# decadenza/SimpleStereo

Measured on AMD Instinct MI355X. Metric: disparity MPixels/s (H*W*nDisp per second), higher is better.
Workload: dtype f32

## Files before the change

simplestereo_amd/csrc/asw_exact_kernels.hip.h:

```cpp
#pragma once
#include "asw_shared.hip.h"
#include "lab_kernels.hip.h"
#include "glibc_math.hip.h"

namespace ssamd {

struct AswExactArgs {
    const PixRec *recL, *recR;
    const double *labL, *labR;
    const double *prox;
    u64 *keyL, *keyR;
    int16_t *disp;
    AswExactQueue q;
    AswExactQueue raw;
    double *ecost;
    u64 *costL, *costR;
    uint32_t *idxL, *idxR;
    uint32_t *wslotL, *wslotR;
    uint32_t *wpix;
    double *wtab;
    unsigned int wcap;
    int H, W, win, pad, minD, maxD, row0, rows;
    double gammaC;
};

__device__ __forceinline__ double exact_sqrt(double x)
{
#pragma clang fp contract(off)
    const double y0 = sqrt(x);
    if (!(y0 > 0.0) || !(y0 < 1.0e300)) return y0;
    const double e = fma(-y0, y0, x);
    return y0 + e / (2.0 * y0);
}

__global__ __launch_bounds__(256) void bgr2lab_f64_pair_kernel(const PixRec *__restrict__ recL, const PixRec *__restrict__ recR,
                                                               double *__restrict__ labL, double *__restrict__ labR, long long npix)
{
    SSAMD_LAB_TABLES_IN_LDS(T)
    long long q = (long long)blockIdx.x * blockDim.x + threadIdx.x;
    const long long stride = (long long)gridDim.x * blockDim.x;
    for (; q < 2 * npix; q += stride) {
        const bool right = q >= npix;
        const long long p = right ? q - npix : q;
        const uint32_t v = (right ? recR : recL)[p].bgrx;
        double L, a, b;
        bgr_to_lab_f64(v & 0xff, (v >> 8) & 0xff, (v >> 16) & 0xff, L, a, b, T);
        double *const o = (right ? labR : labL) + 3 * p;
        o[0] = L; o[1] = a; o[2] = b;
    }
}

__device__ __forceinline__ bool exact_overflowed(const AswExactArgs &A)
{
    return A.q.counter[0] > A.q.cap || (A.raw.entries && A.raw.counter[0] > A.raw.cap);
}

__global__ __launch_bounds__(256) void asw_exact_filter_kernel(const AswExactArgs A)
{
    const unsigned n = min(A.raw.counter[0], A.raw.cap);
    const unsigned nloop = (n + 255u) & ~255u;
    for (unsigned e0 = blockIdx.x * blockDim.x; e0 < nloop; e0 += gridDim.x * blockDim.x) {
        const unsigned e = e0 + threadIdx.x;
        unsigned s2 = 0;
        uint32_t pix = 0, rkey = 0xffffffffu;
        int d = 0;
        if (e < n) {
            const u64 ent = A.raw.entries[e];
            const uint32_t key = A.raw.ekeys[e];
            rkey = key;
            pix = (uint32_t)ent;
            d = (int)((ent >> 32) & 0xffff);
            const unsigned sides = (unsigned)(ent >> 48) & 3u;
            const uint32_t esc = 0xC0000000u - __float_as_uint(2.0f * A.q.sat_abs);
            if (sides & EXACT_SIDE_L) {
                const u64 g = A.keyL[pix];
                if ((int)(uint32_t)g != d && (uint32_t)(g >> 32) < esc && exact_near(key, (uint32_t)(g >> 32), A.q.tol, A.q.sat_abs, exact_zkey(A.win))) s2 |= EXACT_SIDE_L;
            }
            if ((sides & EXACT_SIDE_R) && A.keyR) {
                const u64 g = A.keyR[pix - (uint32_t)d];
                if ((uint32_t)g != pix % (uint32_t)A.W && (uint32_t)(g >> 32) < esc && exact_near(key, (uint32_t)(g >> 32), A.q.tol, A.q.sat_abs, exact_zkey(A.win))) s2 |= EXACT_SIDE_R;
            }
        }
        asw_exact_push_wave(A.q, s2 != 0, pix, d, s2, rkey);
    }
}

__global__ __launch_bounds__(256) void asw_exact_escalate_kernel(const AswExactArgs A)
{
    const AswExactQueue &Q = A.q;
    const uint32_t esc = 0xC0000000u - __float_as_uint(2.0f * Q.sat_abs);
    const long long n = (long long)A.rows * A.W;
    for (long long q = (long long)blockIdx.x * blockDim.x + threadIdx.x; q < n; q += (long long)gridDim.x * blockDim.x) {
        const int x = (int)(q % A.W);
        const u64 gl = A.keyL[q];
        if (gl != KEY_NONE && (uint32_t)(gl >> 32) >= esc) {
            const int dwin = (int)(uint32_t)gl, dhi = min(A.maxD, x);
            const int cnt = dhi - A.minD;
            if (cnt > 0) {
                unsigned slot = atomicAdd(Q.counter, (unsigned)cnt);
                for (int d = A.minD; d <= dhi; ++d)
                    if (d != dwin) {
                        if (slot < Q.cap) Q.entries[slot] = exact_entry((uint32_t)q, d, EXACT_SIDE_L);
                        ++slot;
                    }
                Q.flagL[q] = 1;
            }
        }
        if (A.keyR) {
            const u64 gr = A.keyR[q];
            if (gr != KEY_NONE && (uint32_t)(gr >> 32) >= esc) {
                const int xwin = (int)(uint32_t)gr;
                const int dhi = min(A.maxD, A.W - 1 - x), cnt = dhi - A.minD;
                if (cnt > 0) {
                    unsigned slot = atomicAdd(Q.counter, (unsigned)cnt);
                    for (int d = A.minD; d <= dhi; ++d)
                        if (x + d != xwin) {
                            if (slot < Q.cap) Q.entries[slot] = exact_entry((uint32_t)(q + d), d, EXACT_SIDE_R);
                            ++slot;
                        }
                    Q.flagR[q] = 1;
                }
            }
        }
    }
}

static constexpr int EXACT_ZSEG = 64, EXACT_ZWIN_MAX = 64;
__global__ __launch_bounds__(256) void asw_exact_zero_kernel(const AswExactArgs A)
{
    extern __shared__ __attribute__((aligned(16))) char zsmem[];
    const AswExactQueue &Q = A.q;
    const int W = A.W, H = A.H, win = A.win, p = A.pad;
    const int segs_per_row = (W + EXACT_ZSEG - 1) / EXACT_ZSEG;
    const int tid = threadIdx.x;
    const int TW = EXACT_ZSEG + 2 * p;
    uint32_t *const tA = reinterpret_cast<uint32_t *>(zsmem);
    uint32_t *const tB = tA + win * TW;
    __shared__ int s_idx[EXACT_ZSEG], s_state[EXACT_ZSEG];
    __shared__ int s_cur;
    for (long long seg = blockIdx.x; seg < (long long)A.rows * segs_per_row; seg += gridDim.x) {
        const int yr = (int)(seg / segs_per_row), x0 = (int)(seg - (long long)yr * segs_per_row) * EXACT_ZSEG, y = A.row0 + yr;
        if (!Q.zrow[yr]) continue;
        for (int side = 0; side < (A.keyR ? 2 : 1); ++side) {
            __syncthreads();
            if (tid < EXACT_ZSEG) {
                const int x = x0 + tid;
                bool z = false;
                int idx = 0;
                if (x < W) {
                    const long long q = (long long)yr * W + x;
                    if (side == 0) {
                        z = Q.zeroL[q] != 0;
                        if (z) {
                            if (A.keyL) { const u64 g = A.keyL[q]; z = g != KEY_NONE && (uint32_t)(g >> 32) == 0u; idx = (int)(uint32_t)g; }
                            else idx = (int)A.disp[q];
                        }
                    } else {
                        z = Q.zeroR[q] != 0;
                        if (z) { const u64 g = A.keyR[q]; z = g != KEY_NONE && (uint32_t)(g >> 32) == 0u; idx = (int)(uint32_t)g; }
                    }
                }
                s_idx[tid] = idx;
                s_state[tid] = z ? 1 : 0;
            }
            if (__syncthreads_or(tid < EXACT_ZSEG && s_state[tid] == 1) == 0) continue;
            if (win >= EXACT_ZWIN_MAX) {
                if (tid < EXACT_ZSEG && s_state[tid] == 1) s_state[tid] = 3;
            } else {
                const PixRec *const imgA = side ? A.recR : A.recL, *const imgB = side ? A.recL : A.recR;
                auto stage = [&](uint32_t *tile, const PixRec *img, int shift) {
                    for (int k0 = 0; k0 < win * TW; k0 += 8 * 256) {
                        uint32_t v[8];
#pragma unroll
                        for (int u = 0; u < 8; ++u) {
                            const int k = k0 + u * 256 + tid, i = k / TW, c = k - i * TW, ii = y - p + i, cc = x0 - p + c + shift;
                            v[u] = (k < win * TW && (unsigned)ii < (unsigned)H && (unsigned)cc < (unsigned)W) ? img[(size_t)ii * W + cc].bgrx : 0x80000000u;
                        }
#pragma unroll
                        for (int u = 0; u < 8; ++u) {
                            const int k = k0 + u * 256 + tid;
                            if (k < win * TW) tile[k] = v[u];
                        }
                    }
                };
                stage(tA, imgA, 0);
                for (;;) {
                    __syncthreads();
                    if (tid == 0) {
                        int cur = -1;
                        for (int k = 0; k < EXACT_ZSEG; ++k)
                            if (s_state[k] == 1) { cur = side ? s_idx[k] - (x0 + k) : s_idx[k]; break; }
                        s_cur = cur;
                    }
                    __syncthreads();
                    const int d = s_cur;
                    if (d < 0) break;
                    const int shift = side ? d : -d;
                    stage(tB, imgB, shift);
                    __syncthreads();
                    const int px = tid & (EXACT_ZSEG - 1), part = tid >> 6;
                    const bool mine = s_state[px] == 1 && (side ? s_idx[px] - (x0 + px) : s_idx[px]) == d;
                    bool nz = false;
                    if (mine) {
                        uint32_t acc = 0;
                        for (int i = part; i < win; i += 4) {
                            const uint32_t *const ra = tA + i * TW + px, *const rb = tB + i * TW + px;
#pragma unroll 8
                            for (int j = 0; j < win; ++j) {
                                const uint32_t a = ra[j], b = rb[j];
                                acc |= ((a | b) >> 31) ? 0u : (a ^ b);
                            }
                        }
                        nz = acc != 0u;
                    }
                    __syncthreads();
                    if (mine && part == 0) s_state[px] = 2;
                    __syncthreads();
                    if (mine && nz) s_state[px] = 3;
                }
            }
            __syncthreads();
            if (tid < EXACT_ZSEG && s_state[tid] == 3) {
                const int xq = x0 + tid, widx = s_idx[tid];
                const long long pq = (long long)yr * W + xq;
                if (side == 0) {
                    const int dhi = min(A.maxD, xq), cnt = dhi - A.minD;
                    if (cnt > 0) {
                        unsigned slot = atomicAdd(Q.counter, (unsigned)cnt);
                        for (int d = A.minD; d <= dhi; ++d)
                            if (d != widx) { if (slot < Q.cap) Q.entries[slot] = exact_entry((uint32_t)pq, d, EXACT_SIDE_L); ++slot; }
                        Q.flagL[pq] = 1;
                    }
                } else {
                    const int dhi = min(A.maxD, W - 1 - xq), cnt = dhi - A.minD;
                    if (cnt > 0) {
                        unsigned slot = atomicAdd(Q.counter, (unsigned)cnt);
                        for (int d = A.minD; d <= dhi; ++d)
                            if (xq + d != widx) { if (slot < Q.cap) Q.entries[slot] = exact_entry((uint32_t)(pq + d), d, EXACT_SIDE_R); ++slot; }
                        Q.flagR[pq] = 1;
                    }
                }
            }
        }
    }
}

__device__ __forceinline__ void exact_assign_wslot(const AswExactArgs &A, bool flagged, u64 mask, uint32_t pix, uint32_t side)
{
    if (mask == 0 || A.wcap == 0) return;
    const int leader = (int)__builtin_ctzll(mask);
    const unsigned lane = __builtin_amdgcn_mbcnt_hi(~0u, __builtin_amdgcn_mbcnt_lo(~0u, 0u));
    unsigned base = 0;
    if ((int)lane == leader) base = atomicAdd(A.q.counter + 6, (unsigned)__builtin_popcountll(mask));
    base = (unsigned)__builtin_amdgcn_readlane((int)base, leader);
    if (flagged) {
        const unsigned slot = base + (unsigned)__builtin_popcountll(mask & (((u64)1 << lane) - 1));
        (side ? A.wslotR : A.wslotL)[pix] = slot;
        if (slot < A.wcap) A.wpix[slot] = pix | (side << 31);
    }
}

__global__ __launch_bounds__(256) void asw_exact_winners_kernel(const AswExactArgs A)
{
    const AswExactQueue &Q = A.q;
    const long long n = (long long)A.rows * A.W;
    for (long long q0 = (long long)blockIdx.x * blockDim.x; q0 < n; q0 += (long long)gridDim.x * blockDim.x) {
        const long long q = q0 + threadIdx.x;
        const bool inb = q < n;
        const bool fl = inb && Q.flagL[q];
        if (fl) {
            A.costL[q] = ~0ull;
            A.idxL[q] = 0xffffffffu;
        }
        const int dwin = fl ? (A.keyL ? (int)(uint32_t)A.keyL[q] : (int)A.disp[q]) : 0;
        const u64 ml = __builtin_amdgcn_ballot_w64(fl);
        if (ml && fl && (int)__builtin_ctzll(ml) == (int)(threadIdx.x & 63)) atomicAdd(Q.counter + 1, (unsigned)__builtin_popcountll(ml));
        exact_assign_wslot(A, fl, ml, (uint32_t)q, 0u);
        asw_exact_push_wave(Q, fl, (uint32_t)q, dwin, EXACT_SIDE_L, fl && A.keyL ? (uint32_t)(A.keyL[q] >> 32) : 0xffffffffu);
        if (A.keyR) {
            const bool fr = inb && Q.flagR[q];
            int xl = 0, xr = 0;
            if (fr) {
                A.costR[q] = ~0ull;
                A.idxR[q] = 0xffffffffu;
                xr = (int)(q % A.W);
                xl = (int)(uint32_t)A.keyR[q];
            }
            const u64 mr = __builtin_amdgcn_ballot_w64(fr);
            if (mr && fr && (int)__builtin_ctzll(mr) == (int)(threadIdx.x & 63)) atomicAdd(Q.counter + 2, (unsigned)__builtin_popcountll(mr));
            exact_assign_wslot(A, fr, mr, (uint32_t)q, 1u);
            asw_exact_push_wave(Q, fr, (uint32_t)(q + (xl - xr)), xl - xr, EXACT_SIDE_R, fr ? (uint32_t)(A.keyR[q] >> 32) : 0xffffffffu);
        }
    }
}

__global__ __launch_bounds__(256) void asw_exact_wtab_kernel(const AswExactArgs A)
{
#pragma clang fp contract(off)
    __shared__ uint64_t s_exp[256];
    for (int k = threadIdx.x; k < 256; k += blockDim.x) s_exp[k] = gm_exp_tab[k];
    __syncthreads();
    if (exact_overflowed(A)) return;
    const unsigned n = min(A.q.counter[6], A.wcap);
    const int lane = threadIdx.x & 63, W = A.W, H = A.H, win = A.win, p = A.pad, win2 = win * win;
    for (unsigned slot = blockIdx.x * 4 + (threadIdx.x >> 6); slot < n; slot += gridDim.x * 4) {
        const uint32_t pw = A.wpix[slot], pix = pw & 0x7fffffffu;
        const double *const lab = (pw >> 31) ? A.labR : A.labL;
        const int yr = (int)(pix / (uint32_t)W), x = (int)(pix - (uint32_t)yr * (uint32_t)W), y = A.row0 + yr;
        const double *const c = lab + 3 * ((size_t)y * W + x);
        const double c0 = c[0], c1 = c[1], c2 = c[2];
        double *const out = A.wtab + (size_t)slot * win2;
        for (int t = lane; t < win2; t += 64) {
            const int i = t / win, j = t - i * win, ii = y - p + i, cc = x - p + j;
            double w = 0.0;
            if ((unsigned)ii < (unsigned)H && (unsigned)cc < (unsigned)W) {
                const double *const tp = lab + 3 * ((size_t)ii * W + cc);
                const double a0 = tp[0] - c0, a1 = tp[1] - c1, a2 = tp[2] - c2;
                w = A.prox[t] * glibc_exp_t(-exact_sqrt(a0 * a0 + a1 * a1 + a2 * a2) / A.gammaC, s_exp);
            }
            out[t] = w;
        }
    }
}

static constexpr int EXACT_WAVES = 4;
static constexpr int EXACT_CHUNK = 256;
__global__ __launch_bounds__(64 * EXACT_WAVES) void asw_exact_eval_kernel(const AswExactArgs A)
{
#pragma clang fp contract(off)
    __shared__ double s_w[EXACT_WAVES][EXACT_CHUNK], s_c[EXACT_WAVES][EXACT_CHUNK];
    __shared__ uint64_t s_exp[256];
    for (int k = threadIdx.x; k < 256; k += blockDim.x) s_exp[k] = gm_exp_tab[k];
    __syncthreads();
    if (exact_overflowed(A)) return;
    const int lane = threadIdx.x & 63, wv = threadIdx.x >> 6;
    double *const sw = s_w[wv], *const sc = s_c[wv];
    const unsigned n = min(A.q.counter[0], A.q.cap);
    const int W = A.W, H = A.H, win = A.win, p = A.pad;
    for (unsigned e = blockIdx.x * EXACT_WAVES + wv; e < n; e += gridDim.x * EXACT_WAVES) {
        const u64 ent = A.q.entries[e];
        const uint32_t pix = (uint32_t)ent;
        const int d = (int)((ent >> 32) & 0xffff);
        const unsigned sides = (unsigned)(ent >> 48) & 3u;
        const int yr = (int)(pix / (uint32_t)W), x = (int)(pix - (uint32_t)yr * (uint32_t)W);
        const int y = A.row0 + yr, xr = x - d;
        const double *const cl = A.labL + 3 * ((size_t)y * W + x), *const cr = A.labR + 3 * ((size_t)y * W + xr);
        const double cl0 = cl[0], cl1 = cl[1], cl2 = cl[2], cr0 = cr[0], cr1 = cr[1], cr2 = cr[2];
        const int jlo = max(0, p - xr), jhi = min(win, W + p - x), ncol = jhi - jlo;
        const int ilo = max(0, p - y), ihi = min(win, H + p - y);
        const int ntap = (ihi - ilo) * ncol;
        const uint32_t s1 = A.wcap && A.q.flagL && A.q.flagL[pix] ? A.wslotL[pix] : 0xffffffffu;
        const uint32_t s2 = A.wcap && A.q.flagR && A.q.flagR[pix - (uint32_t)d] ? A.wslotR[pix - (uint32_t)d] : 0xffffffffu;
        const double *const t1 = s1 < A.wcap ? A.wtab + (size_t)s1 * win * win : nullptr;
        const double *const t2 = s2 < A.wcap ? A.wtab + (size_t)s2 * win * win : nullptr;
        double acc = 0.0;
        bool all_zero = false;
        if ((unsigned)(ent >> 48) & EXACT_HINT_ZERO) {
            bool nz = false;
            for (int t = lane; t < ntap; t += 64) {
                const int q = t / ncol, i = ilo + q, j = jlo + (t - q * ncol);
                const int ii = y - p + i, jj = xr - p + j, kk = x - p + j;
                nz = nz || __builtin_amdgcn_sad_u8(A.recL[(size_t)ii * W + kk].bgrx, A.recR[(size_t)ii * W + jj].bgrx, 0u) != 0u;
            }
            all_zero = __builtin_amdgcn_ballot_w64(nz) == 0;
        }
        for (int t0 = 0; t0 < (all_zero ? 0 : ntap); t0 += EXACT_CHUNK) {
            const int nt = min(EXACT_CHUNK, ntap - t0);
            for (int t = lane; t < nt; t += 64) {
                const int q = (t0 + t) / ncol, i = ilo + q, j = jlo + (t0 + t - q * ncol);
                const int ii = y - p + i, jj = xr - p + j, kk = x - p + j;
                const double pr = A.prox[i * win + j];
                double w1, w2;
                if (t1) w1 = t1[i * win + j];
                else {
                    const double *const tl = A.labL + 3 * ((size_t)ii * W + kk);
                    const double a0 = tl[0] - cl0, a1 = tl[1] - cl1, a2 = tl[2] - cl2;
                    w1 = pr * glibc_exp_t(-exact_sqrt(a0 * a0 + a1 * a1 + a2 * a2) / A.gammaC, s_exp);
                }
                if (t2) w2 = t2[i * win + j];
                else {
                    const double *const tr = A.labR + 3 * ((size_t)ii * W + jj);
                    const double b0 = tr[0] - cr0, b1 = tr[1] - cr1, b2 = tr[2] - cr2;
                    w2 = pr * glibc_exp_t(-exact_sqrt(b0 * b0 + b1 * b1 + b2 * b2) / A.gammaC, s_exp);
                }
                const int tad = min(40, (int)__builtin_amdgcn_sad_u8(A.recL[(size_t)ii * W + kk].bgrx, A.recR[(size_t)ii * W + jj].bgrx, 0u));
                const double ww = w1 * w2;
                sw[t] = ww;
                sc[t] = ww * tad;
            }
            __builtin_amdgcn_wave_barrier();
            asm volatile("s_waitcnt lgkmcnt(0)" ::: "memory");
            if (lane < 2) {
                const double *const src = lane ? sw : sc;
                int t = 0;
                for (; t + 16 <= nt; t += 16) {
                    double v[16];
#pragma unroll
                    for (int u = 0; u < 16; ++u) v[u] = src[t + u];
#pragma unroll
                    for (int u = 0; u < 16; ++u) acc += v[u];
                }
                for (; t < nt; ++t) acc += src[t];
            }
            asm volatile("s_waitcnt lgkmcnt(0)" ::: "memory");
            __builtin_amdgcn_wave_barrier();
        }
        const double tot = __shfl(acc, 1);
        if (lane == 0) {
            const double c = all_zero ? 0.0 : acc / tot;
            A.ecost[e] = c;
            const u64 bits = (u64)__double_as_longlong(c);
            if (sides & EXACT_SIDE_L) atomicMin(A.costL + pix, bits);
            if (sides & EXACT_SIDE_R) atomicMin(A.costR + (pix - (uint32_t)d), bits);
        }
    }
}

__global__ __launch_bounds__(256) void asw_exact_resolve_kernel(const AswExactArgs A)
{
    if (exact_overflowed(A)) return;
    const unsigned n = A.q.counter[0];
    for (unsigned e = blockIdx.x * blockDim.x + threadIdx.x; e < n; e += gridDim.x * blockDim.x) {
        const u64 ent = A.q.entries[e];
        const uint32_t pix = (uint32_t)ent;
        const int d = (int)((ent >> 32) & 0xffff);
        const unsigned sides = (unsigned)(ent >> 48) & 3u;
        const u64 bits = (u64)__double_as_longlong(A.ecost[e]);
        if ((sides & EXACT_SIDE_L) && A.costL[pix] == bits) atomicMin(A.idxL + pix, (uint32_t)d);
        if ((sides & EXACT_SIDE_R) && A.costR[pix - (uint32_t)d] == bits) atomicMin(A.idxR + (pix - (uint32_t)d), pix % (uint32_t)A.W);
    }
}

__global__ __launch_bounds__(256) void asw_exact_patch_kernel(const AswExactArgs A)
{
    if (exact_overflowed(A)) return;
    const long long n = (long long)A.rows * A.W;
    for (long long q = (long long)blockIdx.x * blockDim.x + threadIdx.x; q < n; q += (long long)gridDim.x * blockDim.x) {
        if (A.q.flagL[q] && A.idxL[q] != 0xffffffffu) {
            if (A.keyL) A.keyL[q] = (A.keyL[q] & 0xffffffff00000000ull) | (u64)A.idxL[q];
            else A.disp[q] = (int16_t)A.idxL[q];
        }
        if (A.keyR && A.q.flagR[q] && A.idxR[q] != 0xffffffffu) A.keyR[q] = (A.keyR[q] & 0xffffffff00000000ull) | (u64)A.idxR[q];
    }
}

}
```

simplestereo_amd/csrc/host_asw_exact.h:

```cpp
namespace {
int get_prox64(Ctx &c, int win, double gammaP, hipStream_t s, const double **out);

int asw_exact_prepare(Ctx &c, int W, int rows, int win, int nD, double gammaC, bool consistent, bool direct, hipStream_t s,
                      AswExactQueue &q, AswExactQueue &raw, AswExactQueue &kernel_q)
{
    const size_t nout = (size_t)rows * W;
    if (nout >= ((size_t)1 << 32)) return fail(SSAMD_ELIMIT, "exact mode: more than 2^32 output pixels per call");
    const size_t all_cands = 2 * (nout * (size_t)nD + nout);
    size_t cap = std::min<size_t>(std::max<size_t>(4 * nout, std::min<size_t>(all_cands, (size_t)1 << 23)), (size_t)1 << 26);
    if (tune().exact_cap) cap = (size_t)tune().exact_cap;
    size_t rawcap = direct ? 0 : std::min<size_t>(std::max<size_t>(2 * nout, std::min<size_t>(all_cands, (size_t)1 << 23)), (size_t)1 << 26);
    if (!direct && tune().exact_cap) rawcap = std::max<size_t>(rawcap, cap);
    if (!direct && tune().exact_rawcap) rawcap = (size_t)tune().exact_rawcap;
    int rc;
    if ((rc = c.xqueue.reserve(cap * 8)) || (rc = c.xcost.reserve(cap * 8)) || (rc = c.xflags.reserve(64 + 4 * nout + (size_t)rows)) ||
        (rc = c.xslots.reserve(nout * 32)) || (rawcap && (rc = c.xraw.reserve(rawcap * 12))))
        return rc;
    c.xcap = (unsigned int)cap;
    c.xrawcap = (unsigned int)rawcap;
    HIP_TRY(hipMemsetAsync(c.xflags.ptr, 0, 64 + 4 * nout + (size_t)rows, s));
    q.entries = (u64 *)c.xqueue.ptr;
    q.ekeys = nullptr;
    q.counter = (unsigned int *)c.xflags.ptr;
    q.flagL = (unsigned char *)c.xflags.ptr + 64;
    q.flagR = consistent ? q.flagL + nout : nullptr;
    q.zeroL = q.flagL + 2 * nout;
    q.zeroR = consistent ? q.flagL + 3 * nout : nullptr;
    q.zrow = q.flagL + 4 * nout;
    q.W = (unsigned int)W;
    q.cap = (unsigned int)cap;
    q.tol = (uint32_t)std::min(1.0e6, (double)tune().exact_tol * std::max(1.0, 5.0 / gammaC) * std::max(1.0, win / 35.0));
    q.sat_abs = (float)(1.5 * 2.0 * 2.0 * ((double)win * win + 3.0) * 1.1102230246251565e-16 * 40.0);
    q.deep = 0xffffffffu;
    raw = AswExactQueue{};
    if (!direct) {
        raw = q;
        union { float f; uint32_t u; } sa; sa.f = q.sat_abs;
        raw.deep = 0xC0000000u - sa.u;
        raw.entries = (u64 *)c.xraw.ptr;
        raw.ekeys = (uint32_t *)((u64 *)c.xraw.ptr + rawcap);
        raw.counter = q.counter + 4;
        raw.flagL = raw.flagR = nullptr;
        raw.cap = (unsigned int)rawcap;
    }
    kernel_q = direct ? q : raw;
    return SSAMD_OK;
}

int asw_exact_pass(Ctx &c, const AswExactQueue &q, const AswExactQueue &raw, int H, int W, int row0, int rows, int win, int maxD, int minD, double gammaC, double gammaP,
                   bool consistent, bool direct, int16_t *d_disp, hipStream_t s)
{
    const int p = win / 2;
    const size_t nout = (size_t)rows * W, npix = (size_t)H * W;
    int rc;
    const double *d_prox = nullptr;
    if ((rc = get_prox64(c, win, gammaP, s, &d_prox))) return rc;
    if ((rc = c.xlabL.reserve(npix * 24)) || (rc = c.xlabR.reserve(npix * 24))) return rc;
    AswExactArgs x;
    x.recL = (const PixRec *)c.recL.ptr; x.recR = (const PixRec *)c.recR.ptr;
    x.labL = (const double *)c.xlabL.ptr; x.labR = (const double *)c.xlabR.ptr;
    x.prox = d_prox;
    x.keyL = direct ? nullptr : (u64 *)c.keyL.ptr; x.keyR = consistent ? (u64 *)c.keyR.ptr : nullptr;
    x.disp = d_disp;
    x.q = q;
    x.raw = raw;
    x.ecost = (double *)c.xcost.ptr;
    x.costL = (u64 *)c.xslots.ptr; x.costR = x.costL + nout;
    x.idxL = (uint32_t *)(x.costR + nout); x.idxR = x.idxL + nout;
    x.wslotL = x.idxR + nout; x.wslotR = x.wslotL + nout;
    {
        const size_t per = (size_t)win * win * 8;
        size_t wcap = std::min<size_t>(65536, ((size_t)64 << 20) / per);
        if (nout >= ((size_t)1 << 31)) wcap = 0;
        if (wcap && (rc = c.xwtab.reserve(wcap * 8 + wcap * per))) return rc;
        x.wcap = (unsigned int)wcap;
        x.wpix = (uint32_t *)c.xwtab.ptr;
        x.wtab = (double *)((char *)c.xwtab.ptr + wcap * 8);
    }
    x.H = H; x.W = W; x.win = win; x.pad = p; x.minD = minD; x.maxD = maxD; x.row0 = row0; x.rows = rows;
    x.gammaC = gammaC;
    Timed t(c, s, SSAMD_K_ASW_EXACT);
    {
        const int r0 = std::max(0, row0 - p), r1 = std::min(H, row0 + rows + p);
        const long long np2 = (long long)(r1 - r0) * W;
        const int blocks = (int)std::min<long long>((2 * np2 + 255) / 256, 256 * 8);
        hipLaunchKernelGGL(bgr2lab_f64_pair_kernel, dim3(blocks), dim3(256), 0, s, x.recL + (size_t)r0 * W, x.recR + (size_t)r0 * W,
                           (double *)c.xlabL.ptr + 3 * (size_t)r0 * W, (double *)c.xlabR.ptr + 3 * (size_t)r0 * W, np2);
    }
    const int pb = (int)std::min<long long>(((long long)nout + 255) / 256, 256 * 8);
    if (raw.entries) {
        hipLaunchKernelGGL(asw_exact_filter_kernel, dim3(256 * 8), dim3(256), 0, s, x);
        hipLaunchKernelGGL(asw_exact_escalate_kernel, dim3(pb), dim3(256), 0, s, x);
    }
    {
        const int zwin = std::min(win, EXACT_ZWIN_MAX - 1);
        const size_t zlds = (size_t)2 * zwin * (EXACT_ZSEG + 2 * (zwin / 2)) * 4;
        if ((rc = grant_dyn_lds(c, (const void *)asw_exact_zero_kernel, (int)zlds))) return rc;
        const long long segs = (long long)rows * ((W + EXACT_ZSEG - 1) / EXACT_ZSEG);
        hipLaunchKernelGGL(asw_exact_zero_kernel, dim3((unsigned)std::min<long long>(segs, 256 * 64)), dim3(256), zlds, s, x);
    }
    hipLaunchKernelGGL(asw_exact_winners_kernel, dim3(pb), dim3(256), 0, s, x);
    if (x.wcap) hipLaunchKernelGGL(asw_exact_wtab_kernel, dim3(256 * 4), dim3(256), 0, s, x);
    hipLaunchKernelGGL(asw_exact_eval_kernel, dim3((unsigned)(c.cus * 5)), dim3(64 * EXACT_WAVES), 0, s, x);
    hipLaunchKernelGGL(asw_exact_resolve_kernel, dim3(256 * 4), dim3(256), 0, s, x);
    hipLaunchKernelGGL(asw_exact_patch_kernel, dim3(pb), dim3(256), 0, s, x);
    HIP_TRY(hipGetLastError());
    ++c.exact_calls;
    return SSAMD_OK;
}

int asw_exact_counters(Ctx &c, unsigned int (&ctr)[5])
{
    std::fill(ctr, ctr + 5, 0u);
    if (!c.xflags.ptr || c.exact_calls == 0) return SSAMD_OK;
    HIP_TRY(hipDeviceSynchronize());
    HIP_TRY(hipMemcpy(ctr, c.xflags.ptr, sizeof(ctr), hipMemcpyDeviceToHost));
    return SSAMD_OK;
}
}
```

Baseline: 10980.

## Software-pipeline tap loads in exact ASW eval and size grid by occupancy

Restructures the exact eval kernel so each chunk's global loads (Lab values, prox, BGR records, or cached weight table entries) go into registers ahead of time. The next chunk is prefetched while the two-lane reduction of the current one runs. The chunk size drops to one wave-width, and center colors and table slots are forced uniform with readfirstlane. The grid size now comes from an occupancy query instead of a fixed multiple of CUs. This aims to hide memory latency behind the serial reduction, at the cost of more register pressure and extra clamped loads on tail lanes.

```diff
diff --git a/simplestereo_amd/csrc/asw_exact_kernels.hip.h b/simplestereo_amd/csrc/asw_exact_kernels.hip.h
--- a/simplestereo_amd/csrc/asw_exact_kernels.hip.h
+++ b/simplestereo_amd/csrc/asw_exact_kernels.hip.h
@@ -324,7 +324,23 @@
 }
 
 static constexpr int EXACT_WAVES = 4;
-static constexpr int EXACT_CHUNK = 256;
+static constexpr int EXACT_CHUNK = 64;
+static constexpr int EXACT_TRIPS = EXACT_CHUNK / 64;
+
+__device__ __forceinline__ double exact_uniform(double v)
+{
+    const long long b = __double_as_longlong(v);
+    const uint32_t lo = (uint32_t)__builtin_amdgcn_readfirstlane((int)(uint32_t)b), hi = (uint32_t)__builtin_amdgcn_readfirstlane((int)(uint32_t)((u64)b >> 32));
+    return __longlong_as_double((long long)(((u64)hi << 32) | lo));
+}
+
+struct ExactTaps {
+    double pr[EXACT_TRIPS];
+    double l0[EXACT_TRIPS], l1[EXACT_TRIPS], l2[EXACT_TRIPS];
+    double r0[EXACT_TRIPS], r1[EXACT_TRIPS], r2[EXACT_TRIPS];
+    uint32_t bl[EXACT_TRIPS], br[EXACT_TRIPS];
+};
+
 __global__ __launch_bounds__(64 * EXACT_WAVES) void asw_exact_eval_kernel(const AswExactArgs A)
 {
 #pragma clang fp contract(off)
@@ -333,7 +349,7 @@
     for (int k = threadIdx.x; k < 256; k += blockDim.x) s_exp[k] = gm_exp_tab[k];
     __syncthreads();
     if (exact_overflowed(A)) return;
-    const int lane = threadIdx.x & 63, wv = threadIdx.x >> 6;
+    const int lane = threadIdx.x & 63, wv = __builtin_amdgcn_readfirstlane((int)(threadIdx.x >> 6));
     double *const sw = s_w[wv], *const sc = s_c[wv];
     const unsigned n = min(A.q.counter[0], A.q.cap);
     const int W = A.W, H = A.H, win = A.win, p = A.pad;
@@ -345,12 +361,13 @@
         const int yr = (int)(pix / (uint32_t)W), x = (int)(pix - (uint32_t)yr * (uint32_t)W);
         const int y = A.row0 + yr, xr = x - d;
         const double *const cl = A.labL + 3 * ((size_t)y * W + x), *const cr = A.labR + 3 * ((size_t)y * W + xr);
-        const double cl0 = cl[0], cl1 = cl[1], cl2 = cl[2], cr0 = cr[0], cr1 = cr[1], cr2 = cr[2];
+        const double cl0 = exact_uniform(cl[0]), cl1 = exact_uniform(cl[1]), cl2 = exact_uniform(cl[2]);
+        const double cr0 = exact_uniform(cr[0]), cr1 = exact_uniform(cr[1]), cr2 = exact_uniform(cr[2]);
         const int jlo = max(0, p - xr), jhi = min(win, W + p - x), ncol = jhi - jlo;
         const int ilo = max(0, p - y), ihi = min(win, H + p - y);
         const int ntap = (ihi - ilo) * ncol;
-        const uint32_t s1 = A.wcap && A.q.flagL && A.q.flagL[pix] ? A.wslotL[pix] : 0xffffffffu;
-        const uint32_t s2 = A.wcap && A.q.flagR && A.q.flagR[pix - (uint32_t)d] ? A.wslotR[pix - (uint32_t)d] : 0xffffffffu;
+        const uint32_t s1 = __builtin_amdgcn_readfirstlane(A.wcap && A.q.flagL && A.q.flagL[pix] ? A.wslotL[pix] : 0xffffffffu);
+        const uint32_t s2 = __builtin_amdgcn_readfirstlane(A.wcap && A.q.flagR && A.q.flagR[pix - (uint32_t)d] ? A.wslotR[pix - (uint32_t)d] : 0xffffffffu);
         const double *const t1 = s1 < A.wcap ? A.wtab + (size_t)s1 * win * win : nullptr;
         const double *const t2 = s2 < A.wcap ? A.wtab + (size_t)s2 * win * win : nullptr;
         double acc = 0.0;
@@ -364,32 +381,54 @@
             }
             all_zero = __builtin_amdgcn_ballot_w64(nz) == 0;
         }
-        for (int t0 = 0; t0 < (all_zero ? 0 : ntap); t0 += EXACT_CHUNK) {
+        ExactTaps T;
+        auto load_chunk = [&](int t0) {
+#pragma unroll
+            for (int u = 0; u < EXACT_TRIPS; ++u) {
+                const int t = min(t0 + lane + 64 * u, ntap - 1);
+                const int q = t / ncol, i = ilo + q, j = jlo + (t - q * ncol);
+                const int ii = y - p + i, jj = xr - p + j, kk = x - p + j;
+                const size_t al = (size_t)ii * W + kk, ar = (size_t)ii * W + jj;
+                T.pr[u] = A.prox[i * win + j];
+                const double *const tl = t1 ? t1 + (i * win + j) : A.labL + 3 * al, *const tr = t2 ? t2 + (i * win + j) : A.labR + 3 * ar;
+                T.l0[u] = tl[0];
+                if (!t1) { T.l1[u] = tl[1]; T.l2[u] = tl[2]; }
+                T.r0[u] = tr[0];
+                if (!t2) { T.r1[u] = tr[1]; T.r2[u] = tr[2]; }
+                T.bl[u] = A.recL[al].bgrx;
+                T.br[u] = A.recR[ar].bgrx;
+            }
+        };
+        const int ntap_run = all_zero ? 0 : ntap;
+        if (ntap_run > 0) load_chunk(0);
+        for (int t0 = 0; t0 < ntap_run; t0 += EXACT_CHUNK) {
             const int nt = min(EXACT_CHUNK, ntap - t0);
-            for (int t = lane; t < nt; t += 64) {
-                const int q = (t0 + t) / ncol, i = ilo + q, j = jlo + (t0 + t - q * ncol);
-                const int ii = y - p + i, jj = xr - p + j, kk = x - p + j;
-                const double pr = A.prox[i * win + j];
-                double w1, w2;
-                if (t1) w1 = t1[i * win + j];
-                else {
-                    const double *const tl = A.labL + 3 * ((size_t)ii * W + kk);
-                    const double a0 = tl[0] - cl0, a1 = tl[1] - cl1, a2 = tl[2] - cl2;
-                    w1 = pr * glibc_exp_t(-exact_sqrt(a0 * a0 + a1 * a1 + a2 * a2) / A.gammaC, s_exp);
-                }
-                if (t2) w2 = t2[i * win + j];
-                else {
-                    const double *const tr = A.labR + 3 * ((size_t)ii * W + jj);
-                    const double b0 = tr[0] - cr0, b1 = tr[1] - cr1, b2 = tr[2] - cr2;
-                    w2 = pr * glibc_exp_t(-exact_sqrt(b0 * b0 + b1 * b1 + b2 * b2) / A.gammaC, s_exp);
-                }
-                const int tad = min(40, (int)__builtin_amdgcn_sad_u8(A.recL[(size_t)ii * W + kk].bgrx, A.recR[(size_t)ii * W + jj].bgrx, 0u));
-                const double ww = w1 * w2;
-                sw[t] = ww;
-                sc[t] = ww * tad;
+#pragma unroll
+            for (int u = 0; u < EXACT_TRIPS; ++u) {
+                if (64 * u < nt) {
+                    const int t = lane + 64 * u;
+                    double w1, w2;
+                    if (t1) w1 = T.l0[u];
+                    else {
+                        const double a0 = T.l0[u] - cl0, a1 = T.l1[u] - cl1, a2 = T.l2[u] - cl2;
+                        w1 = T.pr[u] * glibc_exp_t(-exact_sqrt(a0 * a0 + a1 * a1 + a2 * a2) / A.gammaC, s_exp);
+                    }
+                    if (t2) w2 = T.r0[u];
+                    else {
+                        const double b0 = T.r0[u] - cr0, b1 = T.r1[u] - cr1, b2 = T.r2[u] - cr2;
+                        w2 = T.pr[u] * glibc_exp_t(-exact_sqrt(b0 * b0 + b1 * b1 + b2 * b2) / A.gammaC, s_exp);
+                    }
+                    const int tad = min(40, (int)__builtin_amdgcn_sad_u8(T.bl[u], T.br[u], 0u));
+                    const double ww = w1 * w2;
+                    if (t < nt) {
+                        sw[t] = ww;
+                        sc[t] = ww * tad;
+                    }
+                }
             }
             __builtin_amdgcn_wave_barrier();
             asm volatile("s_waitcnt lgkmcnt(0)" ::: "memory");
+            if (t0 + EXACT_CHUNK < ntap) load_chunk(t0 + EXACT_CHUNK);
             if (lane < 2) {
                 const double *const src = lane ? sw : sc;
                 int t = 0;
diff --git a/simplestereo_amd/csrc/host_asw_exact.h b/simplestereo_amd/csrc/host_asw_exact.h
--- a/simplestereo_amd/csrc/host_asw_exact.h
+++ b/simplestereo_amd/csrc/host_asw_exact.h
@@ -44,6 +44,18 @@
         raw.cap = (unsigned int)rawcap;
     }
     kernel_q = direct ? q : raw;
+    return SSAMD_OK;
+}
+
+int asw_exact_eval_groups(Ctx &c, int *groups)
+{
+    static int per_cu[16] = {0};
+    int &n = per_cu[c.dev];
+    if (n <= 0) {
+        HIP_TRY(hipOccupancyMaxActiveBlocksPerMultiprocessor(&n, asw_exact_eval_kernel, 64 * EXACT_WAVES, 0));
+        if (n <= 0) return fail(SSAMD_EHIP, "asw_exact_eval_kernel: no workgroup fits a compute unit");
+    }
+    *groups = c.cus * n;
     return SSAMD_OK;
 }
 
@@ -101,7 +113,9 @@
     }
     hipLaunchKernelGGL(asw_exact_winners_kernel, dim3(pb), dim3(256), 0, s, x);
     if (x.wcap) hipLaunchKernelGGL(asw_exact_wtab_kernel, dim3(256 * 4), dim3(256), 0, s, x);
-    hipLaunchKernelGGL(asw_exact_eval_kernel, dim3((unsigned)(c.cus * 5)), dim3(64 * EXACT_WAVES), 0, s, x);
+    int eval_groups = 0;
+    if ((rc = asw_exact_eval_groups(c, &eval_groups))) return rc;
+    hipLaunchKernelGGL(asw_exact_eval_kernel, dim3((unsigned)eval_groups), dim3(64 * EXACT_WAVES), 0, s, x);
     hipLaunchKernelGGL(asw_exact_resolve_kernel, dim3(256 * 4), dim3(256), 0, s, x);
     hipLaunchKernelGGL(asw_exact_patch_kernel, dim3(pb), dim3(256), 0, s, x);
     HIP_TRY(hipGetLastError());
```

Result: no change. 10990, median of 4 (+0.0%).
